# Angtian/VoGE

Measured on AMD Instinct MI355X. Metric: forward+backward frames/sec at 512^2, 50k Gaussians; ray-trace HBM GB/s vs peak, higher is better.
Workload: dtype f32; 1 GPU; cfg3_50k_512: 50000 random Gaussians (scalar sigmas), 512x512, K=40, max_point_per_bin=-1, fwd+bwd (grads to verts, sigmas, colors); launch=hip graph replay, 4 consecutive steps per graph launch, parallelism=1 gpu

## Files before the change

voge_amd/csrc/sweep_iso.h:

```cpp
#pragma once
#include <type_traits>

#include "voge_common.h"

namespace voge {

constexpr int kS2TP = 65;
constexpr int kS2TQ = 66;
constexpr int kS2Pad = 4;

struct Sweep2Stage {
  float x[64 + kS2Pad], y[64 + kS2Pad], z[64 + kS2Pad], a[64 + kS2Pad];
  union {
    float lb[64];
    int cnt[64];
  };
  int pos[64 + kS2Pad];
};
__host__ __device__ constexpr size_t sweep2_len_bytes(const int K) { return (sizeof(float) * (size_t)(K + 1) * kS2TP + 15) & ~(size_t)15; }
__host__ __device__ constexpr size_t sweep2_pos_bytes(const int K) { return (sizeof(uint16_t) * (size_t)(K + 1) * kS2TQ + 15) & ~(size_t)15; }
struct Sweep2Gen {
  float e[11][64 + kS2Pad];
};
constexpr int kS2DiagRows = 5;
__host__ __device__ constexpr size_t sweep2_lds_bytes(const int K, const int gen = 0) {
  return sweep2_len_bytes(K) + sweep2_pos_bytes(K) + sizeof(Sweep2Stage) +
         (gen == 1 ? sizeof(Sweep2Gen) : (gen == 2 ? sizeof(float) * kS2DiagRows * (64 + kS2Pad) : 0));
}

#ifndef VOGE_S2_EPI_B
#define VOGE_S2_EPI_B 5
#endif
#ifndef VOGE_S2_EPI_R
#define VOGE_S2_EPI_R 3
#endif
#ifndef VOGE_S2_EXIT_GROUP
#define VOGE_S2_EXIT_GROUP 16
#endif
constexpr int kExitGroup = VOGE_S2_EXIT_GROUP;

template <int GEN>
__global__ void __launch_bounds__(64)
sweep_iso_kernel(const float4 *__restrict__ cull, const float4 *__restrict__ ms, const float4 *__restrict__ evr, const float *__restrict__ rays,
                 const int *__restrict__ bin_count, const int32_t *__restrict__ bin_id, const float *__restrict__ bin_lb,
                 const int32_t *__restrict__ tl_id, const float *__restrict__ tl_lb, const int32_t *__restrict__ pool_id,
                 const float *__restrict__ pool_lb, const int *__restrict__ tl_off, const int2 *__restrict__ order,
                 const int tiles_per_img, const int nstx, const int nst, const int N, const int H, const int W, const int K,
                 const float thr_act, int32_t *__restrict__ out_idx, float *__restrict__ out_len, float *__restrict__ out_act,
                 float *__restrict__ out_dsd, int32_t *__restrict__ out_cnt,
                 const CamView cam ) {
  extern __shared__ __attribute__((aligned(16))) unsigned char smem_raw[];
  float *const Llen = reinterpret_cast<float *>(smem_raw);
  unsigned char *const Lpos_raw = smem_raw + sweep2_len_bytes(K);
  Sweep2Stage &S = *reinterpret_cast<Sweep2Stage *>(smem_raw + sweep2_len_bytes(K) + sweep2_pos_bytes(K));
  Sweep2Gen &G = *reinterpret_cast<Sweep2Gen *>(smem_raw + sweep2_len_bytes(K) + sweep2_pos_bytes(K) + sizeof(Sweep2Stage));
  auto grow = [&](const int r) -> float * { return &G.e[GEN == 2 ? (r < 2 ? r : r - 3) : r][0]; };
  auto ghas = [](const int r) { return GEN != 2 || r < 2 || (r >= 5 && r < 8); };

  const int lane = threadIdx.x;
  const int tiles_x = (W + 7) >> 3;
#ifdef VOGE_SWEEP_TIMES
  const unsigned long long ts0 = wall_clock64();
  unsigned long long ts_fill = 0, ts_cons = 0, ts1 = 0, ts2 = 0;
  unsigned st_eval = 0;
  unsigned long long ts_slow = 0; unsigned st_slow = 0, st_lanes = 0, st_moved = 0, st_far = 0;
  int dbg_moved = 0;
#endif
  const int2 slot = order[blockIdx.x];
  if (slot.x < 0) return;
  if (slot.y == 0) {
    if (out_act != nullptr) return;
    const int lin0 = slot.x & ~kPoolFlag;
    const int b = lin0 / tiles_per_img, bx = lin0 - b * tiles_per_img;
    const int ftx = bx % tiles_x, fty = bx / tiles_x;
    const int tw = min(8, W - ftx * 8), th = min(8, H - fty * 8);
    const int row_items = tw * K;
    if ((K & 3) == 0) {
      const int ipr = row_items >> 2;
      for (int it = lane; it < th * ipr; it += 64) {
        const int rr = it / ipr, j4 = it - rr * ipr;
        const size_t o = (((size_t)b * H + fty * 8 + rr) * W + (size_t)ftx * 8) * K + (size_t)j4 * 4;
        st16i<true>(out_idx + o, -1, -1, -1, -1);
        st16f<true>(out_len + o, VOGE_SENT_LEN, VOGE_SENT_LEN, VOGE_SENT_LEN, VOGE_SENT_LEN);
      }
    } else {
      for (int it = lane; it < th * row_items; it += 64) {
        const int rr = it / row_items, j = it - rr * row_items;
        const size_t o = (((size_t)b * H + fty * 8 + rr) * W + (size_t)ftx * 8) * K + j;
        out_idx[o] = -1; out_len[o] = VOGE_SENT_LEN;
      }
    }
    if (out_cnt != nullptr) {
      const int rr = lane >> 3, x = lane & 7;
      if (rr < th && x < tw) out_cnt[((size_t)b * H + fty * 8 + rr) * W + (size_t)ftx * 8 + x] = 0;
// ... 7 lines not shown
        float *o = cam.rays_out + (((size_t)b * H + fty * 8 + rr) * W + (size_t)ftx * 8 + x) * 3;
        o[0] = ex; o[1] = ey; o[2] = ez;
      }
    }
    return;
  }
  const bool pooled = (slot.x & kPoolFlag) != 0;
  const int lin = slot.x & ~kPoolFlag;
  const int b = lin / tiles_per_img, bx = lin - b * tiles_per_img;
  const int tx = bx % tiles_x, ty = bx / tiles_x;
  const int bin = (b * nst + ((ty * 8) / kST) * nstx + (tx * 8) / kST) * 4 + (((ty * 8) / kQuad) & 1) * 2 + (((tx * 8) / kQuad) & 1);
  const int tc = slot.y;
  const int bc = (tc >= 0) ? tc : ((bin_count != nullptr) ? bin_count[bin] : -1);
  const bool binned = bc >= 0;
  const int src_n = binned ? bc : N;
  const size_t list_at = pooled ? (size_t)tl_off[lin] : (size_t)lin * kTileCap;
  const int32_t *src_id = (tc >= 0) ? (pooled ? pool_id : tl_id) + list_at : (binned ? bin_id + (size_t)bin * kQCap : nullptr);
  const float *src_lb = (tc >= 0) ? (pooled ? pool_lb : tl_lb) + list_at : (binned ? bin_lb + (size_t)bin * kQCap : nullptr);
  const bool pref = tc >= 0;
  const float4 *cullb = cull + (size_t)b * N;
  const float4 *msb = ms + (size_t)b * N;
  const float4 rec_none = make_float4(0.f, 0.f, 0.f, INFINITY);
  const float4 cull_none = make_float4(0.f, 0.f, 0.f, -1.f);
  const bool h_is_id = (N <= 65536) || !binned;
  auto id_of = [&](const unsigned h) -> int { return h_is_id ? (int)h : src_id[h]; };
  const float not_full = __uint_as_float(__float_as_uint(VOGE_SENT_LEN) - 1u);
  if (lane < kS2Pad) { S.x[64 + lane] = 0.f; S.y[64 + lane] = 0.f; S.z[64 + lane] = 0.f; S.a[64 + lane] = INFINITY; }
  if (GEN && lane < kS2Pad) G.e[0][64 + lane] = __uint_as_float(0x7fc00000u);
  const float4 *evrb = GEN ? evr + (size_t)b * N * 3 : nullptr;
  bool tile_gen = false;

  Cone wcone;
  bool unit_rays = false;
  wcone.ok = false;
  const bool from_cam = cam.R != nullptr;
  CamK ck;
  if (from_cam) ck = cam_load(cam, b);
  auto ray_of = [&](const int x, const int y, float &rx, float &ry, float &rz) {
    if (from_cam) {
      cam_ray(ck, cam_irow(cam, y), x, rx, ry, rz);
    } else {
      const size_t rid = ((size_t)b * H + y) * W + x;
      rx = rays[3 * rid + 0]; ry = rays[3 * rid + 1]; rz = rays[3 * rid + 2];
    }
  };
  auto ray_setup = [&](const bool mine, const float mdx, const float mdy, const float mdz) {
    const int px = tx * 8 + (lane & 7), py = ty * 8 + (lane >> 3);
    float ox_ = mdx, oy_ = mdy, oz_ = mdz;
    if (!mine) ray_of(min(px, W - 1), min(py, H - 1), ox_, oy_, oz_);
    const RayDir u = ray_dir(ox_, oy_, oz_);
    unit_rays = __all(!u.ok || u.unit);
    wcone.ok = false;
    if (!pref) {
      const bool dirs_ok = __all(u.ok);
      const float wsx = wave_sum_dpp(u.ok ? u.ux : 0.f), wsy = wave_sum_dpp(u.ok ? u.uy : 0.f), wsz = wave_sum_dpp(u.ok ? u.uz : 0.f);
      const float n = sqrtf(fmaf(wsz, wsz, fmaf(wsy, wsy, wsx * wsx)));
      const float ax = wsx / n, ay = wsy / n, az = wsz / n;
      float smax = 0.f, cmin = 1.f;
      cone_partial(u, ax, ay, az, smax, cmin);
      wcone = cone_finish(ax, ay, az, n, wave_max(smax), wave_min(cmin), dirs_ok);
    }
  };

  auto run = [&](auto wide_tag, const int pass) {
    constexpr bool WIDE = decltype(wide_tag)::value;
    const int r = WIDE ? pass * 32 + (lane & 31) : lane;
    const int col = WIDE ? (lane & 31) : lane;
    const int px = tx * 8 + (r & 7), py = ty * 8 + (r >> 3);
    const bool valid = (px < W) && (py < H) && (!WIDE || lane < 32);
    const size_t ray_id = ((size_t)b * H + min(py, H - 1)) * W + min(px, W - 1);
    int id0 = (lane < src_n) ? (binned ? src_id[lane] : lane) : -1;
    float lb0 = (binned && lane < src_n) ? src_lb[lane] : -INFINITY;
    int id1 = (64 + lane < src_n) ? (binned ? src_id[64 + lane] : 64 + lane) : -1;
    float lb1 = (binned && 64 + lane < src_n) ? src_lb[64 + lane] : -INFINITY;
    float dx, dy, dz;
    ray_of(min(px, W - 1), min(py, H - 1), dx, dy, dz);
    if (from_cam && cam.rays_out != nullptr && valid) {
      float *o = cam.rays_out + 3 * ray_id;
      o[0] = dx; o[1] = dy; o[2] = dz;
    }
    const __amdgpu_buffer_rsrc_t rs_ms = out_rsrc(const_cast<float4 *>(msb), (unsigned)N * 16u),
                                 rs_cull = out_rsrc(const_cast<float4 *>(cullb), (unsigned)N * 16u);
    auto load_ms = [&](const int id) {
      const voge_v4f r = __builtin_amdgcn_raw_buffer_load_b128(rs_ms, id * 16, 0, 0);
      return make_float4(r[0], r[1], r[2], (id >= 0) ? r[3] : INFINITY);
    };
    auto load_cull = [&](const int id) {
      const voge_v4f r = __builtin_amdgcn_raw_buffer_load_b128(rs_cull, id * 16, 0, 0);
      return make_float4(r[0], r[1], r[2], (id >= 0) ? r[3] : -1.f);
    };
    const __amdgpu_buffer_rsrc_t rs_ev = out_rsrc(const_cast<float4 *>(GEN ? evrb : msb), GEN ? (unsigned)N * 48u : 0u);
    auto load_ev = [&](const int id, const int k) {
      const voge_v4f r = __builtin_amdgcn_raw_buffer_load_b128(rs_ev, id * 48 + 16 * k, 0, 0);
      return make_float4(r[0], r[1], r[2], r[3]);
    };
    float4 m0 = load_ms(id0);
    float4 c0 = pref ? cull_none : load_cull(id0);
    float4 ea0 = rec_none, ea1 = rec_none, ea2 = rec_none;
    if (GEN) { ea0 = load_ev(id0, 0); ea1 = load_ev(id0, 1); ea2 = load_ev(id0, 2); }
    if (pass == 0) ray_setup(!WIDE, dx, dy, dz);
    const float rdn2 = __builtin_amdgcn_rcpf((dx * dx + dy * dy) + dz * dz);
    float *const mylen = Llen + col;
// ... 333 lines not shown
        Pn = *reinterpret_cast<const int4 *>(&S.pos[s0 + 4]);
        if (GEN && chunk_diag) {
#pragma unroll
          for (int r = 0; r < 11; ++r)
            if (r < 2 || (r >= 5 && r < 8)) Evn[GEN ? r : 0] = *reinterpret_cast<const float4 *>(grow(r) + s0 + 4);
        } else if (GEN == 1 && gmask != 0ull) {
#pragma unroll
          for (int r = 0; r < 11; ++r) Evn[GEN ? r : 0] = *reinterpret_cast<const float4 *>(&G.e[r][s0 + 4]);
        }
#pragma unroll
        for (int q = 0; q < 4; ++q) commit(len[q], act[q], (unsigned)pv[q]);
      }
#ifdef VOGE_SWEEP_TIMES
      ts_cons += wall_clock64() - tsb;
      st_eval += min(n, nbuf);
#endif
    }
#ifdef VOGE_SWEEP_TIMES
    ts2 = wall_clock64();
#endif

    __syncthreads();
    S.cnt[lane] = valid ? cnt : 0;
    if (out_cnt != nullptr && valid) out_cnt[((size_t)b * H + py) * W + px] = cnt;
    __syncthreads();
    const int row0 = WIDE ? pass * 4 : 0;
    const int th = max(0, min(WIDE ? 4 : 8, H - ty * 8 - row0)), tw = min(8, W - tx * 8);
    const int row_items = tw * K;
    const uint16_t *const P16 = reinterpret_cast<const uint16_t *>(Lpos_raw);
    const uint32_t *const P32 = reinterpret_cast<const uint32_t *>(Lpos_raw);
    auto entry_pos = [&](const int s, const int owner) -> unsigned {
      return WIDE ? P32[s * (kS2TQ / 2) + owner] : (unsigned)P16[s * kS2TQ + owner];
    };
    const bool want_ad = out_act != nullptr;
    const int gofs = b * N;
    if ((K & 3) == 0) {
      constexpr int kEpiB = VOGE_S2_EPI_B, kEpiR = VOGE_S2_EPI_R;
      const int ipr = row_items >> 2, nitem = th * ipr;
      const float inv_ipr = 1.0f / (float)max(ipr, 1), invK = 1.0f / (float)K;
      const size_t tile_pix = ((size_t)b * H + ty * 8 + row0) * W + (size_t)tx * 8;
      int32_t *const t_idx = out_idx + tile_pix * K;
      float *const t_len = out_len + tile_pix * K;
      const unsigned h_last = (unsigned)max(src_n - 1, 0);
      const bool wt_ok = (size_t)W * (size_t)K < ((size_t)1 << 26);
      const unsigned rs_bytes = wt_ok ? (unsigned)th * (unsigned)W * (unsigned)K * 4u : 0u;
      const __amdgpu_buffer_rsrc_t rs_idx = out_rsrc(t_idx, rs_bytes), rs_len = out_rsrc(t_len, rs_bytes);
      for (int it0 = lane; it0 < nitem; it0 += 64 * kEpiB) {
        int32_t oi[kEpiB][4];
        float ol[kEpiB][4];
        unsigned rel[kEpiB];
        int nv[kEpiB];
#pragma unroll
        for (int u = 0; u < kEpiB; ++u) {
          const int it = it0 + u * 64;
          const bool in = it < nitem;
          const int itc = in ? it : 0;
          const int rr = __float2int_rz(((float)itc + 0.5f) * inv_ipr);
          const int j = (itc - rr * ipr) * 4;
          const int x = __float2int_rz(((float)j + 0.5f) * invK);
          const int sl = j - x * K;
          const int owner = rr * 8 + x;
          rel[u] = (unsigned)(rr * W + x) * (unsigned)K + (unsigned)sl;
          nv[u] = in ? max(0, min(4, S.cnt[owner] - sl)) : -1;
#pragma unroll
          for (int q = 0; q < 4; ++q) {
            const float l = Llen[(sl + q) * kS2TP + owner];
            const unsigned h = entry_pos(sl + q, owner);
// ... 147 lines not shown
#pragma unroll
          for (int u = 0; u < kOddU; ++u) {
            const float *ry = rays + (tile_pix + pr[u]) * 3;
            const float ex = ry[0], ey = ry[1], ez = ry[2];
            const size_t gi = (size_t)(in[u] ? oi[u] : gofs);
            const float4 cc = ms[gi];
            PairOut o;
            if (GEN && tile_gen && !(cc.w == cc.w)) {
              o = pair_eval_gen(cc.x, cc.y, cc.z, unpack_eval(evr[gi * 3], evr[gi * 3 + 1], evr[gi * 3 + 2]), ex, ey, ez, ex * ex, ey * ey,
                                ez * ez, ex * ey, ex * ez, ey * ez);
            } else {
              o = pair_eval_iso_at(cc.x, cc.y, cc.z, cc.w, ol[u], ex, ey, ez, (ex * ex + ey * ey) + ez * ez);
            }
            oa[u] = in[u] ? o.act : VOGE_SENT_ACT; od[u] = in[u] ? o.dsd : 0.0f;
          }
#pragma unroll
          for (int u = 0; u < kOddU; ++u)
            if (on[u]) { t_idx[rel[u]] = oi[u]; t_len[rel[u]] = ol[u]; t_act[rel[u]] = oa[u]; t_dsd[rel[u]] = od[u]; }
        }
      }
    }
  };

  if ((h_is_id ? N : src_n) <= 65536) {
    run(std::false_type{}, 0);
  } else {
    run(std::true_type{}, 0);
    run(std::true_type{}, 1);
  }
#ifdef VOGE_SWEEP_TIMES
  if (lane == 0 && b == 0 && bx < 8192) {
    unsigned long long *o = g_sweep_times + 8 * (size_t)bx;
    o[0] = ts0; o[1] = ts1; o[2] = ts_fill; o[3] = ts_cons; o[4] = ts2; o[5] = wall_clock64(); o[6] = ((unsigned long long)blockIdx.x << 32) | st_eval;
#ifdef VOGE_SWEEP_SLOW
    o[7] = (ts_slow << 32) | st_slow;
    o[2] = ((unsigned long long)st_far << 48) | ((unsigned long long)(st_moved & 0xffffu) << 32) | st_lanes;
#else
    o[7] = (unsigned long long)__builtin_amdgcn_s_getreg((4 << 0) | (0 << 6) | (31 << 11)) |
           ((unsigned long long)__builtin_amdgcn_s_getreg((20 << 0) | (0 << 6) | (31 << 11)) << 32);
#endif
  }
#endif
}

}
```

voge_amd/csrc/trace_bin.h:

```cpp
#pragma once
#include <type_traits>

#include "voge_common.h"

namespace voge {

constexpr int kST0 = 128;
constexpr int kCh = kST0 / kST;
constexpr int kBinThreads = 1024;
constexpr int kParts = 16;
constexpr int kSegCap = 512;
constexpr int kTileCap = 2048;
constexpr int kTilesPerBin = (kST / 8) * (kST / 8);
constexpr int kRankMaxBins = 4096;
static_assert(kCh * kCh == kBinThreads / 64, "one wave per super-tile of a region / per sweep tile of a super-tile");

__device__ __forceinline__ float depth_key(const float4 c, const Cone &k) {
  const float nm = __builtin_amdgcn_sqrtf(fmaf(c.z, c.z, fmaf(c.y, c.y, c.x * c.x)));
  const float R = c.w;
  if (!(R < 3e38f) || !(nm < 3e38f)) return -INFINITY;
  float kappa = -nm;
  if (k.ok && k.cs >= 0.5f && nm > 4.0f * R) {
    const float p = fmaf(c.z, k.az, fmaf(c.y, k.ay, c.x * k.ax));
    if (p > 0.0f) kappa = nm;
// ... 118 lines not shown
            const CamView cam ) {
  __shared__ BinALds L;
  const int tid = threadIdx.x, lane = tid & 63, wave = tid >> 6;
  const int region = blockIdx.x / kParts, part = blockIdx.x - region * kParts;
  const int b = blockIdx.y;
  if (blockIdx.x == 0 && blockIdx.y == 0 && tid == 0) *pool_top = 0ull;
  const int rx = region % nst0x, ry = region / nst0x;
  const int nst = nstx * nsty;
  if (tid < kCh * kCh) { L.base[tid] = 0; L.extn[tid] = 0; }
  if (tid == 0) L.arena_top = 0;
  int32_t *const arena = ext_id + ((size_t)(b * (int)(gridDim.x / kParts) + region) * kParts + part) * (size_t)ext_arena;
  int ext_have = 0;
  BIN_TS(0, 0);
  const bool interleaved = deal_interleaved(N);
  const int nchunks = interleaved ? kParts * ((N + kParts * kBinThreads - 1) / (kParts * kBinThreads))
                                  : (N + kBinThreads - 1) / kBinThreads;
  const bool writes_records = ISO_PREP && region == 0;
  float4 c[kRoundChunks];
  float av[kRoundChunks];
  int gq[kRoundChunks];
  CamK ck;
  if (cam.R != nullptr) ck = cam_load(cam, b);
  const BinAView V = binA_view<ISO_PREP>(b, cam_fwd, view, cam, &ck);
  if (cam.R != nullptr && cam.origin_out != nullptr && blockIdx.x == 0 && tid == 0) {
    float ox = V.ox, oy = V.oy, oz = V.oz;
    if (!ISO_PREP) cam_origin(ck, cam.T + 3 * b, ox, oy, oz);
    cam.origin_out[3 * b] = ox; cam.origin_out[3 * b + 1] = oy; cam.origin_out[3 * b + 2] = oz;
  }
  BinARaw raw[kRoundChunks];
  auto fetch_round = [&](const int j0) {
#pragma unroll
    for (int q = 0; q < kRoundChunks; ++q) {
      const int j = j0 + q * kParts;
      const int g = interleaved ? ((j / kParts) * kBinThreads + tid) * kParts + part : j * kBinThreads + tid;
      gq[q] = (j < nchunks && g < N) ? g : -1;
      raw[q] = binA_fetch<ISO_PREP>(gq[q], b, N, cull, mus, isg, view);
    }
  };
  auto derive_round = [&]() {
#pragma unroll
    for (int q = 0; q < kRoundChunks; ++q) c[q] = binA_derive<ISO_PREP>(raw[q], gq[q] >= 0, V, thr_act, view, av[q]);
  };
  auto load_round = [&](const int j0) { fetch_round(j0); derive_round(); };
  fetch_round(part);
  if (wave == 0) {
    const int cc = lane & (kCh * kCh - 1);
    const int cx = rx * kCh + (cc & (kCh - 1)), cy = ry * kCh + cc / kCh;
    ConeRec r = {0.f, 0.f, 1.f, 1.f, 0.f, -1.f, 0.f, 0.f};
    const bool region_rect = cam.R != nullptr && cam.h <= cam.stripe_h;
    if (cam.R != nullptr) {
      const bool reg = region_rect && lane == kCh * kCh;
      const int j0 = reg ? rx * kCh * kST : cx * kST, i0 = reg ? ry * kCh * kST : cy * kST, ext = reg ? kCh * kST : kST;
      if ((cx < nstx && cy < nsty) || reg) r = cam_rect_cone(ck, cam, j0, j0 + ext - 1, i0, i0 + ext - 1);
    } else if (cx < nstx && cy < nsty) {
      r = cones[cone_super_at(b, nst, cy * nstx + cx)];
    }
    if (lane < kCh * kCh) L.child[lane] = r;
    if (region_rect) {
      if (lane == kCh * kCh) L.region = r;
      if (lane == 0) L.use_rows = 0;
    } else {
    const bool present = lane < kCh * kCh && r.ok >= 0.f;
    const float sx = wave_sum_dpp(present ? r.ax : 0.f), sy = wave_sum_dpp(present ? r.ay : 0.f), sz = wave_sum_dpp(present ? r.az : 0.f);
    const float npres = wave_sum_dpp(present ? 1.f : 0.f);
    bool ok = __all(!present || r.ok > 0.f);
    const float n = sqrtf(fmaf(sz, sz, fmaf(sy, sy, sx * sx)));
    const float ax = sx / n, ay = sy / n, az = sz / n;
    auto child_extrema = [&](const float ax_, const float ay_, const float az_, float &smax_, float &cmin_, bool &ok_) {
      smax_ = 0.f; cmin_ = 1.f;
      if (present) {
        const float ca = fmaf(r.az, az_, fmaf(r.ay, ay_, r.ax * ax_));
        const float qx = fmaf(-ca, ax_, r.ax), qy = fmaf(-ca, ay_, r.ay), qz = fmaf(-ca, az_, r.az);
        const float sa = sqrtf(fmaf(qz, qz, fmaf(qy, qy, qx * qx))) * (1.0f + 1e-6f) + 1e-7f;
        const float cl = fminf(ca, 1.0f) - 1e-7f;
        if (!(cl > 0.0f)) ok_ = false;
        cmin_ = fmaf(cl, r.cs, -sa * r.sn);
        smax_ = fmaf(fminf(ca + 1e-7f, 1.0f), r.sn, sa);
      }
    };
    float smax, cmin;
    child_extrema(ax, ay, az, smax, cmin, ok);
    ok = __all(ok);
    smax = wave_max(smax); cmin = wave_min(cmin);
    const Cone cn = cone_finish(ax, ay, az, n / fmaxf(npres, 1.f), smax, cmin, ok);
    if (lane == 0) L.region = ConeRec{cn.ax, cn.ay, cn.az, cn.cs, cn.sn, cn.ok ? 1.f : 0.f, 0.f, 0.f};
    const float widest_child = wave_max(present ? (r.ok > 0.f ? r.sn : 2.0f) : 0.f);
    if (lane == 0) L.use_rows = 0;
    if (__builtin_expect((!cn.ok || cn.sn > 8.0f * widest_child) && N < (1 << 27), 0)) {
      auto quad_sum = [](float v) { v += VOGE_DPP(v, 0xB1); v += VOGE_DPP(v, 0x4E); return v; };
      auto quad_max = [](float v) { v = fmaxf(v, VOGE_DPP(v, 0xB1)); v = fmaxf(v, VOGE_DPP(v, 0x4E)); return v; };
      auto quad_min = [](float v) { v = fminf(v, VOGE_DPP(v, 0xB1)); v = fminf(v, VOGE_DPP(v, 0x4E)); return v; };
      static_assert(kCh == 4, "a row of super-tiles is a DPP quad");
      const float qsx = quad_sum(present ? r.ax : 0.f), qsy = quad_sum(present ? r.ay : 0.f), qsz = quad_sum(present ? r.az : 0.f);
      const float qn = quad_sum(present ? 1.f : 0.f);
      const float nn = sqrtf(fmaf(qsz, qsz, fmaf(qsy, qsy, qsx * qsx)));
      const float rax = qsx / nn, ray = qsy / nn, raz = qsz / nn;
      float rs, rc;
      bool rok = !present || r.ok > 0.f;
      child_extrema(rax, ray, raz, rs, rc, rok);
      rs = quad_max(rs); rc = quad_min(rc);
      const float okf = quad_min(rok ? 1.f : 0.f);
      const Cone rcn = cone_finish(rax, ray, raz, nn / fmaxf(qn, 1.f), rs, rc, okf != 0.f);
      if (lane < kCh * kCh && (lane & 3) == 0) L.rowc[lane >> 2] = ConeRec{rcn.ax, rcn.ay, rcn.az, rcn.cs, rcn.sn, qn > 0.f ? (rcn.ok ? 1.f : 0.f) : -1.f, 0.f, 0.f};
      const float widest_row = wave_max((lane < kCh * kCh && qn > 0.f) ? (rcn.ok ? rcn.sn : 2.0f) : 0.f);
      if (lane == 0) L.use_rows = (!cn.ok || cn.sn > 1.6f * widest_row) ? 1 : 0;
    }
    }
  }
  BIN_TS(0, 6);
  derive_round();
  BIN_TS(0, 7);
  __syncthreads();
  const Cone rcone = load_cone(L.region);
  const bool use_rows = L.use_rows != 0;
  BIN_TS(0, 1);

  auto rounds = [&](auto rows_tag) {
    constexpr bool ROWS = decltype(rows_tag)::value;
    for (int j0 = part; j0 < nchunks; j0 += kParts * kRoundChunks) {
      if (j0 != part) load_round(j0);
      bool k0[kRoundChunks];
      unsigned rowm[kRoundChunks];
  #pragma unroll
      for (int q = 0; q < kRoundChunks; ++q) {
        if (writes_records && gq[q] >= 0) {
// ... 246 lines not shown
      }
      bin_test_batch<ELL>(S, gid, c, sink);
    }
  }
}
__device__ __forceinline__ void bin_batch_slots(int *count , const int lane, const bool (&kp)[kGU], int (&slot)[kGU]) {
  unsigned long long m[kGU];
  int cw = 0;
#pragma unroll
  for (int j = 0; j < kGU; ++j) { m[j] = __ballot(kp[j]); cw += __popcll(m[j]); }
  int start = 0;
  if (cw > 0) {
    if (lane == 0) start = atomicAdd(count, cw);
    start = __builtin_amdgcn_readfirstlane(start);
  }
#pragma unroll
  for (int j = 0; j < kGU; ++j) {
    slot[j] = start + __popcll(m[j] & ((1ull << lane) - 1ull));
    start += __popcll(m[j]);
  }
}
struct BinKeys {
  float lo, scale, span, slack;
  bool flagged;
};
__device__ __forceinline__ int bin_bucket_of(const BinKeys &Kk, const float v) {
  return (v > -INFINITY) ? 1 + min(kBuckets - 2, max(0, (int)((v - Kk.lo) * Kk.scale))) : 0;
}
__device__ __forceinline__ float bin_own_bound(const BinStream &S, const size_t g) {
  const float4 cj = S.cullb[g], e0 = S.ellb[2 * g], e1 = S.ellb[2 * g + 1];
  float bnd = -INFINITY;
  if (S.qcone.ok) {
    const float pa = fmaf(cj.z, S.qcone.az, fmaf(cj.y, S.qcone.ay, cj.x * S.qcone.ax));
    const float nm1 = fabsf(cj.x) + fabsf(cj.y) + fabsf(cj.z);
    const float t = pa - ell_support(e0, e1, S.qcone.ax, S.qcone.ay, S.qcone.az) - 4e-6f * nm1;
    bnd = (t >= 0.0f) ? t : t / S.qcone.cs;
    bnd = bnd - 1e-5f * fabsf(bnd) - 1e-30f;
  }
  return bnd;
}
__device__ __forceinline__ void bin_bmin_suffix(uint32_t *bmin, int *wsum, const int tid) {
  const int lane = tid & 63, wave = tid >> 6;
  uint32_t m4[2];
#pragma unroll
  for (int q = 0; q < 2; ++q) m4[q] = bmin[2 * tid + q];
  m4[0] = min(m4[0], m4[1]);
  uint32_t x = m4[0];
#pragma unroll
  for (int o = 1; o < 64; o <<= 1) {
    const uint32_t y = __shfl_down(x, o, 64);
    if (lane + o < 64) x = min(x, y);
  }
  if (lane == 0) wsum[4 + wave] = (int)x;
  __syncthreads();
  uint32_t later = 0xffffffffu;
  {
    const uint32_t nxt = __shfl_down(x, 1, 64);
    later = (lane < 63) ? nxt : 0xffffffffu;
    for (int w = wave + 1; w < 4; ++w) later = min(later, (uint32_t)wsum[4 + w]);
  }
#pragma unroll
  for (int q = 0; q < 2; ++q) bmin[2 * tid + q] = min(m4[q], later);
}
__device__ __forceinline__ float bin_len_bound(const BinKeys &Kk, const uint32_t *bmin, const float v) {
  float edge = -INFINITY;
  int qb = 0;
  if (v > -INFINITY) {
    const int q = min(kBuckets - 2, max(0, (int)((v - Kk.lo) * Kk.scale)));
    edge = fminf(v, Kk.lo + (float)q * (Kk.span / (float)(kBuckets - 2)) - 4e-6f * Kk.span);
    qb = 1 + q;
  }
  const float lb_sphere = (edge > -INFINITY) ? edge - Kk.slack - 1e-5f * fabsf(edge) - 1e-30f : -INFINITY;
  return Kk.flagged ? fminf(lb_sphere, ord2f(bmin[qb])) : lb_sphere;
}

struct BinLong {
  BinStream S;
  BinKeys Kk;
  Cone tcone;
  bool tile_ok;
  int tile, quad, total;
  unsigned long long *pool_top;
  int *tl_off, *tl_count, *q_count;
  const int *seg_ext;
  int bin;
  int pool_cap;
  int32_t *pool_id;
  float *pool_lb;
  int2 *my_order;
};
template <bool ELL>
__device__ __forceinline__ void binB_long_path(const BinLong A, BinLds &L) {
// ... 252 lines not shown
        if (!el[j] && cj[j].w < 3e38f) rmax = fmaxf(rmax, cj[j].w);
        const float kv = el[j] ? gkey[j] : depth_key(cj[j], qcone);
        if (kv > -INFINITY) { klo = fminf(klo, kv); khi = fmaxf(khi, kv); }
        if (slot[j] < kQCap) L.keys[slot[j]] = ((uint64_t)f2ord(kv) << 32) | (uint32_t)g[j] | (el[j] ? 0x80000000u : 0u);
        any_el = any_el || el[j];
      }
    }
  });
  BIN_TS(1, 1);
  if (__any(any_el) && lane == 0) L.nflag = 1;
  float hi = wave_max(khi), lo = wave_min(klo), rm = wave_max(rmax);
  if (lane == 0) { L.red[wave * 8 + 0] = hi; L.red[wave * 8 + 1] = lo; L.red[wave * 8 + 2] = rm; }
  if (S.n_ext > 0) __syncthreads();
  for (int i = tid; i < kBuckets; i += kQT) { L.hist[i] = 0; L.bmin[i] = f2ord(INFINITY); }
  __syncthreads();
  const int total = L.count;
  hi = fmaxf(fmaxf(L.red[0], L.red[8]), fmaxf(L.red[16], L.red[24]));
  lo = fminf(fminf(L.red[1], L.red[9]), fminf(L.red[17], L.red[25]));
  rm = fmaxf(fmaxf(L.red[2], L.red[10]), fmaxf(L.red[18], L.red[26]));
  const float span = fmaxf(hi - lo, 1e-20f);
  const float scale = (float)(kBuckets - 2) / span;
  const bool flagged = ELL && L.nflag != 0;
  BinKeys Kk;
  Kk.lo = lo; Kk.scale = scale; Kk.span = span; Kk.slack = 1.13f * rm * (1.0f + 1e-5f); Kk.flagged = flagged;
  auto bucket_of = [&](const uint64_t k) { return bin_bucket_of(Kk, ord2f((uint32_t)(k >> 32))); };
  if (__builtin_expect(total > kQCap, 0)) {
    BinLong A;
    A.S = S; A.Kk = Kk; A.tcone = tcone; A.tile_ok = tile_ok; A.tile = tile; A.quad = quad; A.total = total;
    A.pool_top = pool_top; A.tl_off = tl_off; A.tl_count = tl_count; A.q_count = q_count; A.pool_cap = pool_cap;
    A.pool_id = pool_id; A.pool_lb = pool_lb; A.my_order = my_order; A.seg_ext = seg_ext; A.bin = bin;
    binB_long_path<ELL>(A, L);
  } else {
  for (int i = tid; i < total; i += kQT) {
    const uint64_t kk = L.keys[i];
    const int q = bucket_of(kk);
    atomicAdd(&L.hist[q], 1);
    if (ELL && ((uint32_t)kk & 0x80000000u)) atomicMin(&L.bmin[q], f2ord(bin_own_bound(S, (size_t)((uint32_t)kk & 0x7fffffffu))));
  }
  __syncthreads();
  {
    static_assert(kBuckets == 2 * kQT, "two buckets per thread");
    const int2 v = *reinterpret_cast<const int2 *>(&L.hist[2 * tid]);
    const int s4 = v.x + v.y;
    int x = s4;
#pragma unroll
    for (int o = 1; o < 64; o <<= 1) {
      const int y = __shfl_up(x, o, 64);
// ... 155 lines not shown
```

voge_amd/csrc/trace_fwd.hip:

```cpp
#include "voge_common.h"

namespace voge {

__device__ inline double lambda_min_sym3(double a00, double a11, double a22, double a01,
                                         double a02, double a12) {
  const double p1 = a01 * a01 + a02 * a02 + a12 * a12;
  if (p1 == 0.0) return fmin(a00, fmin(a11, a22));
  const double q = (a00 + a11 + a22) / 3.0;
  const double b00 = a00 - q, b11 = a11 - q, b22 = a22 - q;
  const double p2 = b00 * b00 + b11 * b11 + b22 * b22 + 2.0 * p1;
  const double p = sqrt(p2 / 6.0);
  const double ip = 1.0 / p;
  const double c00 = b00 * ip, c11 = b11 * ip, c22 = b22 * ip;
  const double c01 = a01 * ip, c02 = a02 * ip, c12 = a12 * ip;
  double r = 0.5 * (c00 * (c11 * c22 - c12 * c12) - c01 * (c01 * c22 - c12 * c02) +
                    c02 * (c01 * c12 - c11 * c02));
  r = fmin(1.0, fmax(-1.0, r));
  const double phi = acos(r) / 3.0;
  return q + 2.0 * p * cos(phi + 2.0943951023931953);
}

__device__ __forceinline__ void prep_one(const int g, const float *__restrict__ mus, const float *__restrict__ isg,
                                         const float *__restrict__ cam_fwd, const int N, const float thr_act,
                                         const int iso_in, float4 *__restrict__ cull, float4 *__restrict__ evr,
// ... 307 lines not shown
    ws->tl_lb = reinterpret_cast<float *>(tl);
    ws->seg_rec = reinterpret_cast<float4 *>(sr); ws->order = reinterpret_cast<int2 *>(cq);
    ws->nstx = nstx; ws->nsty = nsty;
    ws->nst0x = (W + kST0 - 1) / kST0; ws->nst0y = (H + kST0 - 1) / kST0;
    ws->nbin = (int)nbin;
  }
  return off;
}

}
#ifdef VOGE_AB
#include "sweep_r3.h"
#else
namespace voge { constexpr bool ab_round3_selected() { return false; } }
#endif
namespace voge {

template <bool ISO>
static int launch_trace(const TraceWs &ws, const ConeRec *cones, const float *rays, int B, int N, int H, int W, int K,
                        float thr_act, int32_t *idx, float *len, float *act, float *dsd, int32_t *cnt, hipStream_t st,
                        const CamView &cam, const bool diag = false) {
  constexpr int T = 64;
  const int gen = ISO ? 0 : (diag ? 2 : 1);
  const auto sweep = ISO ? sweep_iso_kernel<0> : (diag ? sweep_iso_kernel<2> : sweep_iso_kernel<1>);
  const bool v2 = !ab_round3_selected();
  const size_t lds2 = sweep2_lds_bytes(K, gen);
  {
    static DynLdsCache cache2[2];
    if (v2) {
      const int rc = ensure_dynamic_lds(reinterpret_cast<const void *>(sweep), lds2, cache2[diag ? 1 : 0]);
      if (rc) return rc;
    }
  }
  hipLaunchKernelGGL(binB_kernel<!ISO>, dim3(ws.nstx * ws.nsty * 4, B), dim3(kQT), 0, st, ws.cull, ws.ell, ws.seg_count, ws.seg_id, ws.seg_rec,
                     cones, N, H, W, ws.nstx, ws.nsty, ws.nbin, ws.q_count, ws.q_id, ws.q_lb, ws.tl_count, ws.tl_id, ws.tl_lb,
                     ws.order, ws.pool_top, ws.pool_cap, ws.pool_id, ws.pool_lb, ws.tl_off, ws.seg_ext, ws.ext_id, K,
                     (v2 && act == nullptr) ? nullptr : idx , len, act, dsd, cnt,
                     nullptr, nullptr, cam);
  {
    int rc = launch_status();
    if (rc) return rc;
  }
  dim3 grid(ws.nbin * kTilesPerBin);
#ifdef VOGE_AB
  if (!v2) return launch_sweep_r3<ISO>(ws, rays, grid, N, H, W, K, thr_act, idx, len, act, dsd, cnt, st, cam);
#endif
  hipLaunchKernelGGL(sweep, grid, dim3(T), lds2, st, ws.cull, ws.ms, ws.evr, rays, ws.q_count, ws.q_id, ws.q_lb, ws.tl_id,
                     ws.tl_lb, ws.pool_id, ws.pool_lb, ws.tl_off, ws.order, ((W + 7) / 8) * ((H + 7) / 8), ws.nstx, ws.nstx * ws.nsty, N, H, W, K,
                     thr_act, idx, len, act, dsd, cnt, cam);
  return launch_status();
}

}
// ... 367 lines not shown
```

voge_amd/csrc/voge_common.h:

```cpp
#pragma once
#include <hip/hip_runtime.h>
#include <stdint.h>

#include <atomic>
#include <type_traits>

#include "voge_hip.h"

#define VOGE_WAVE 64

#define VOGE_SENT_LEN 1e10f
#define VOGE_SENT_ACT 1e10f

namespace voge {

struct EvalRec {
  float s00, s11, s22, s01, s02, s12;
  float bx, by, bz;
  float kx, ky, kz;
};
static_assert(sizeof(EvalRec) == 48, "EvalRec must be 3 x float4");

__device__ __forceinline__ float fast_div(const float a, const float b) { return a * __builtin_amdgcn_rcpf(b); }

// ... 331 lines not shown
  float ax, ay, az, cs, sn;
  bool ok;
};

__device__ __forceinline__ bool cone_keep(const float4 c, const Cone &k) {
  if (c.w < 0.0f) return false;
  const float p = fmaf(c.z, k.az, fmaf(c.y, k.ay, c.x * k.ax));
  const float rx = fmaf(-p, k.ax, c.x), ry = fmaf(-p, k.ay, c.y), rz = fmaf(-p, k.az, c.z);
  const float q = __builtin_amdgcn_sqrtf(fmaf(rz, rz, fmaf(ry, ry, rx * rx)));
  const float gap = fmaf(q, k.cs, -fabsf(p) * k.sn);
  return !k.ok || !(gap > c.w);
}

constexpr int kST = 32;

struct RayDir {
  float ux, uy, uz;
  bool ok;
  bool unit;
};
__device__ __forceinline__ RayDir ray_dir(const float dx, const float dy, const float dz) {
  RayDir r;
  const float dn2 = fmaf(dz, dz, fmaf(dy, dy, dx * dx));
  const float inv = 1.0f / sqrtf(dn2);
  r.ok = (dn2 > 0.0f) && (inv < 3e38f) && (inv == inv);
  r.unit = fabsf(dn2 - 1.0f) < 1e-4f;
  r.ux = dx * inv; r.uy = dy * inv; r.uz = dz * inv;
  return r;
}
__device__ __forceinline__ void cone_partial(const RayDir &u, const float ax, const float ay, const float az,
                                             float &smax, float &cmin) {
  const float cl = fmaf(u.uz, az, fmaf(u.uy, ay, u.ux * ax));
  const float rx = fmaf(-cl, ax, u.ux), ry = fmaf(-cl, ay, u.uy), rz = fmaf(-cl, az, u.uz);
  const float sl = sqrtf(fmaf(rz, rz, fmaf(ry, ry, rx * rx)));
  smax = fmaxf(smax, u.ok ? sl : 2.0f);
  cmin = fminf(cmin, u.ok ? cl : -1.0f);
}
__device__ __forceinline__ Cone cone_finish(const float ax, const float ay, const float az, const float n,
                                            const float smax, const float cmin, const bool all_ok) {
  Cone c;
  c.ax = ax; c.ay = ay; c.az = az;
  c.sn = smax * (1.0f + 1e-5f) + 1e-7f;
  c.cs = cmin - 1e-6f;
  c.ok = all_ok && (n > 1e-3f) && (cmin > 0.05f) && (c.sn == c.sn);
  return c;
}

struct ConeRec {
  float ax, ay, az, cs, sn, ok, pad0, pad1;
};
__device__ __forceinline__ Cone load_cone(const ConeRec &r) {
  Cone c;
  c.ax = r.ax; c.ay = r.ay; c.az = r.az; c.cs = r.cs; c.sn = r.sn; c.ok = r.ok > 0.f;
  return c;
}

struct Mat3 {
  float m[9];
};
__device__ __forceinline__ Mat3 inv3(const float *R) {
  Mat3 o;
  const float a = R[0], b = R[1], c = R[2], d = R[3], e = R[4], f = R[5], g = R[6], h = R[7], i = R[8];
  const float A = e * i - f * h, B = -(d * i - f * g), C = d * h - e * g;
  const float det = a * A + b * B + c * C;
  const float id = 1.0f / det;
  o.m[0] = A * id;               o.m[1] = -(b * i - c * h) * id;  o.m[2] = (b * f - c * e) * id;
// ... 178 lines not shown
      const float4 v = L.sum[i];
      const float c = L.cnt[i];
      vx += in ? v.x : 0.f; vy += in ? v.y : 0.f; vz += in ? v.z : 0.f;
      ok = (in && c > 0.f) ? fminf(ok, v.w) : ok;
      n_in += in ? c : 0.f;
      const float e_s = level == 0 ? L.ext[i][0] : L.ext[i][2];
      const float e_c = level == 0 ? L.ext[i][1] : L.ext[i][3];
      s2 = (in && c > 0.f && level != 1) ? fmaxf(s2, e_s) : s2;
      cm = (in && c > 0.f && level != 1) ? fminf(cm, e_c) : cm;
    }
    const float n2 = fmaf(vz, vz, fmaf(vy, vy, vx * vx)), rn = __builtin_amdgcn_rsqf(n2);
    const float Ax = vx * rn, Ay = vy * rn, Az = vz * rn;
    float smax = sqrtf(s2) * (1.0f + 4e-7f) + 4e-7f, cmin = cm - 4e-7f;
    bool all_ok = ok != 0.f;
    if (level == 1) {
      smax = 0.f; cmin = 1.f;
#pragma unroll
      for (int k = 0; k < 4; ++k) {
        const int i = q0 + (k >> 1) * 4 + (k & 1);
        if (!(L.cnt[i] > 0.f)) continue;
        const float4 v = L.sum[i];
        const float trn = __builtin_amdgcn_rsqf(fmaf(v.z, v.z, fmaf(v.y, v.y, v.x * v.x)));
        const float tx = v.x * trn, ty = v.y * trn, tz = v.z * trn;
        const float t_sn = (sqrtf(L.ext[i][0]) * (1.0f + 4e-7f) + 4e-7f) * (1.0f + 1e-5f) + 1e-7f;
        const float t_cs = (L.ext[i][1] - 4e-7f) - 1e-6f;
        const float ca = fmaf(tz, Az, fmaf(ty, Ay, tx * Ax));
        const float qx = fmaf(-ca, Ax, tx), qy = fmaf(-ca, Ay, ty), qz = fmaf(-ca, Az, tz);
        const float sa = sqrtf(fmaf(qz, qz, fmaf(qy, qy, qx * qx))) * (1.0f + 1e-6f) + 1e-7f;
        const float cl = fminf(ca, 1.0f) - 1e-7f;
        if (!(cl > 0.0f) || !(t_cs > 0.0f)) all_ok = false;
        cmin = fminf(cmin, fmaf(cl, t_cs, -sa * t_sn));
        smax = fmaxf(smax, fmaf(fminf(ca + 1e-7f, 1.0f), t_sn, sa));
      }
    }
    const Cone c = cone_finish(Ax, Ay, Az, (n2 * rn) / fmaxf(n_in, 1.f), smax, cmin, all_ok);
    const ConeRec rec = {c.ax, c.ay, c.az, c.cs, c.sn, n_in > 0.f ? (c.ok ? 1.f : 0.f) : -1.f, 0.f, 0.f};
    if (level == 0) c_tile[t] = rec; else if (level == 1) c_quad[t - 16] = rec; else *c_super = rec;
  }
}

__device__ __forceinline__ ConeRec cam_rect_cone(const CamK &k, const CamView &c, int j0, int j1, int i0, int i1) {
  if (j0 >= c.W || i0 >= c.h || j1 < j0 || i1 < i0) return ConeRec{0.f, 0.f, 1.f, 1.f, 0.f, -1.f, 0.f, 0.f};
  j1 = min(j1, c.W - 1); i1 = min(i1, c.h - 1);
  const int r0 = cam_irow(c, i0), r1 = cam_irow(c, i1);
  float ux[4], uy[4], uz[4];
  cam_ray(k, r0, j0, ux[0], uy[0], uz[0]); cam_ray(k, r0, j1, ux[1], uy[1], uz[1]);
  cam_ray(k, r1, j0, ux[2], uy[2], uz[2]); cam_ray(k, r1, j1, ux[3], uy[3], uz[3]);
  const float sx = (ux[0] + ux[1]) + (ux[2] + ux[3]), sy = (uy[0] + uy[1]) + (uy[2] + uy[3]), sz = (uz[0] + uz[1]) + (uz[2] + uz[3]);
// ... 320 lines not shown
```

Baseline: 4653 frames/s.

## Specialize iso sweep kernel for frame layout and small N; use fast rsq/sqrt intrinsics

Adds FRAME and HID template specializations of the iso sweep kernel. They compile out the activation/dsd epilogue, drop the id indirection and the wide two-pass path when N is at most 65536, and use byte-offset buffer stores for the ray and count outputs. Separately, divisions and sqrtf in the cone construction and ray normalization become hardware rsq/sqrt/rcp intrinsics, with cone error margins widened to cover the lower precision. A bucket step is precomputed in BinKeys. The wider margins may loosen culling slightly, and the approximate intrinsics change rounding.

```diff
diff --git a/voge_amd/csrc/sweep_iso.h b/voge_amd/csrc/sweep_iso.h
--- a/voge_amd/csrc/sweep_iso.h
+++ b/voge_amd/csrc/sweep_iso.h
@@ -1,6 +1,7 @@
 #pragma once
 #include <type_traits>
 
+#include "composite_core.h"
 #include "voge_common.h"
 
 namespace voge {
@@ -39,7 +40,7 @@
 #endif
 constexpr int kExitGroup = VOGE_S2_EXIT_GROUP;
 
-template <int GEN>
+template <int GEN, bool FRAME = false, bool HID = false>
 __global__ void __launch_bounds__(64)
 sweep_iso_kernel(const float4 *__restrict__ cull, const float4 *__restrict__ ms, const float4 *__restrict__ evr, const float *__restrict__ rays,
                  const int *__restrict__ bin_count, const int32_t *__restrict__ bin_id, const float *__restrict__ bin_lb,
@@ -69,7 +70,7 @@
   const int2 slot = order[blockIdx.x];
   if (slot.x < 0) return;
   if (slot.y == 0) {
-    if (out_act != nullptr) return;
+    if (!FRAME && out_act != nullptr) return;
     const int lin0 = slot.x & ~kPoolFlag;
     const int b = lin0 / tiles_per_img, bx = lin0 - b * tiles_per_img;
     const int ftx = bx % tiles_x, fty = bx / tiles_x;
@@ -123,7 +124,7 @@
   const float4 *msb = ms + (size_t)b * N;
   const float4 rec_none = make_float4(0.f, 0.f, 0.f, INFINITY);
   const float4 cull_none = make_float4(0.f, 0.f, 0.f, -1.f);
-  const bool h_is_id = (N <= 65536) || !binned;
+  const bool h_is_id = HID || (N <= 65536) || !binned;
   auto id_of = [&](const unsigned h) -> int { return h_is_id ? (int)h : src_id[h]; };
   const float not_full = __uint_as_float(__float_as_uint(VOGE_SENT_LEN) - 1u);
   if (lane < kS2Pad) { S.x[64 + lane] = 0.f; S.y[64 + lane] = 0.f; S.z[64 + lane] = 0.f; S.a[64 + lane] = INFINITY; }
@@ -155,11 +156,11 @@
     if (!pref) {
       const bool dirs_ok = __all(u.ok);
       const float wsx = wave_sum_dpp(u.ok ? u.ux : 0.f), wsy = wave_sum_dpp(u.ok ? u.uy : 0.f), wsz = wave_sum_dpp(u.ok ? u.uz : 0.f);
-      const float n = sqrtf(fmaf(wsz, wsz, fmaf(wsy, wsy, wsx * wsx)));
-      const float ax = wsx / n, ay = wsy / n, az = wsz / n;
+      const float n2 = fmaf(wsz, wsz, fmaf(wsy, wsy, wsx * wsx)), rn = __builtin_amdgcn_rsqf(n2);
+      const float ax = wsx * rn, ay = wsy * rn, az = wsz * rn;
       float smax = 0.f, cmin = 1.f;
       cone_partial(u, ax, ay, az, smax, cmin);
-      wcone = cone_finish(ax, ay, az, n, wave_max(smax), wave_min(cmin), dirs_ok);
+      wcone = cone_finish(ax, ay, az, n2 * rn, wave_max(smax), wave_min(cmin), dirs_ok);
     }
   };
 
@@ -176,9 +177,16 @@
     float lb1 = (binned && 64 + lane < src_n) ? src_lb[64 + lane] : -INFINITY;
     float dx, dy, dz;
     ray_of(min(px, W - 1), min(py, H - 1), dx, dy, dz);
+    const size_t tile_pix0 = ((size_t)b * H + ty * 8) * W + (size_t)tx * 8;
+    const unsigned pix_rel = (unsigned)(r >> 3) * (unsigned)W + (unsigned)(r & 7);
     if (from_cam && cam.rays_out != nullptr && valid) {
-      float *o = cam.rays_out + 3 * ray_id;
-      o[0] = dx; o[1] = dy; o[2] = dz;
+      if constexpr (FRAME) {
+        float *const o = cam.rays_out + 3 * tile_pix0;
+        at_bytes_w<float>(o, pix_rel * 12u) = dx; at_bytes_w<float>(o, pix_rel * 12u + 4u) = dy; at_bytes_w<float>(o, pix_rel * 12u + 8u) = dz;
+      } else {
+        float *o = cam.rays_out + 3 * ray_id;
+        o[0] = dx; o[1] = dy; o[2] = dz;
+      }
     }
     const __amdgpu_buffer_rsrc_t rs_ms = out_rsrc(const_cast<float4 *>(msb), (unsigned)N * 16u),
                                  rs_cull = out_rsrc(const_cast<float4 *>(cullb), (unsigned)N * 16u);
@@ -558,7 +566,10 @@
 
     __syncthreads();
     S.cnt[lane] = valid ? cnt : 0;
-    if (out_cnt != nullptr && valid) out_cnt[((size_t)b * H + py) * W + px] = cnt;
+    if (out_cnt != nullptr && valid) {
+      if constexpr (FRAME) at_bytes_w<int32_t>(out_cnt + tile_pix0, pix_rel * 4u) = cnt;
+      else out_cnt[((size_t)b * H + py) * W + px] = cnt;
+    }
     __syncthreads();
     const int row0 = WIDE ? pass * 4 : 0;
     const int th = max(0, min(WIDE ? 4 : 8, H - ty * 8 - row0)), tw = min(8, W - tx * 8);
@@ -568,7 +579,7 @@
     auto entry_pos = [&](const int s, const int owner) -> unsigned {
       return WIDE ? P32[s * (kS2TQ / 2) + owner] : (unsigned)P16[s * kS2TQ + owner];
     };
-    const bool want_ad = out_act != nullptr;
+    const bool want_ad = !FRAME && out_act != nullptr;
     const int gofs = b * N;
     if ((K & 3) == 0) {
       constexpr int kEpiB = VOGE_S2_EPI_B, kEpiR = VOGE_S2_EPI_R;
@@ -578,7 +589,7 @@
       int32_t *const t_idx = out_idx + tile_pix * K;
       float *const t_len = out_len + tile_pix * K;
       const unsigned h_last = (unsigned)max(src_n - 1, 0);
-      const bool wt_ok = (size_t)W * (size_t)K < ((size_t)1 << 26);
+      const bool wt_ok = FRAME || (size_t)W * (size_t)K < ((size_t)1 << 26);
       const unsigned rs_bytes = wt_ok ? (unsigned)th * (unsigned)W * (unsigned)K * 4u : 0u;
       const __amdgpu_buffer_rsrc_t rs_idx = out_rsrc(t_idx, rs_bytes), rs_len = out_rsrc(t_len, rs_bytes);
       for (int it0 = lane; it0 < nitem; it0 += 64 * kEpiB) {
@@ -772,11 +783,15 @@
     }
   };
 
-  if ((h_is_id ? N : src_n) <= 65536) {
+  if constexpr (HID) {
     run(std::false_type{}, 0);
   } else {
-    run(std::true_type{}, 0);
-    run(std::true_type{}, 1);
+    if ((h_is_id ? N : src_n) <= 65536) {
+      run(std::false_type{}, 0);
+    } else {
+      run(std::true_type{}, 0);
+      run(std::true_type{}, 1);
+    }
   }
 #ifdef VOGE_SWEEP_TIMES
   if (lane == 0 && b == 0 && bx < 8192) {
diff --git a/voge_amd/csrc/trace_bin.h b/voge_amd/csrc/trace_bin.h
--- a/voge_amd/csrc/trace_bin.h
+++ b/voge_amd/csrc/trace_bin.h
@@ -164,7 +164,7 @@
   CamK ck;
   if (cam.R != nullptr) ck = cam_load(cam, b);
   const BinAView V = binA_view<ISO_PREP>(b, cam_fwd, view, cam, &ck);
-  if (cam.R != nullptr && cam.origin_out != nullptr && blockIdx.x == 0 && tid == 0) {
+  if ((ISO_PREP || N <= 0) && cam.R != nullptr && cam.origin_out != nullptr && blockIdx.x == 0 && tid == 0) {
     float ox = V.ox, oy = V.oy, oz = V.oz;
     if (!ISO_PREP) cam_origin(ck, cam.T + 3 * b, ox, oy, oz);
     cam.origin_out[3 * b] = ox; cam.origin_out[3 * b + 1] = oy; cam.origin_out[3 * b + 2] = oz;
@@ -206,25 +206,25 @@
     const float sx = wave_sum_dpp(present ? r.ax : 0.f), sy = wave_sum_dpp(present ? r.ay : 0.f), sz = wave_sum_dpp(present ? r.az : 0.f);
     const float npres = wave_sum_dpp(present ? 1.f : 0.f);
     bool ok = __all(!present || r.ok > 0.f);
-    const float n = sqrtf(fmaf(sz, sz, fmaf(sy, sy, sx * sx)));
-    const float ax = sx / n, ay = sy / n, az = sz / n;
+    const float n2 = fmaf(sz, sz, fmaf(sy, sy, sx * sx)), rn = __builtin_amdgcn_rsqf(n2);
+    const float ax = sx * rn, ay = sy * rn, az = sz * rn;
     auto child_extrema = [&](const float ax_, const float ay_, const float az_, float &smax_, float &cmin_, bool &ok_) {
       smax_ = 0.f; cmin_ = 1.f;
       if (present) {
         const float ca = fmaf(r.az, az_, fmaf(r.ay, ay_, r.ax * ax_));
         const float qx = fmaf(-ca, ax_, r.ax), qy = fmaf(-ca, ay_, r.ay), qz = fmaf(-ca, az_, r.az);
-        const float sa = sqrtf(fmaf(qz, qz, fmaf(qy, qy, qx * qx))) * (1.0f + 1e-6f) + 1e-7f;
-        const float cl = fminf(ca, 1.0f) - 1e-7f;
+        const float sa = __builtin_amdgcn_sqrtf(fmaf(qz, qz, fmaf(qy, qy, qx * qx))) * (1.0f + 1e-6f) + 4e-7f;
+        const float cl = fminf(ca, 1.0f) - 4e-7f;
         if (!(cl > 0.0f)) ok_ = false;
         cmin_ = fmaf(cl, r.cs, -sa * r.sn);
-        smax_ = fmaf(fminf(ca + 1e-7f, 1.0f), r.sn, sa);
+        smax_ = fmaf(fminf(ca + 4e-7f, 1.0f), r.sn, sa);
       }
     };
     float smax, cmin;
     child_extrema(ax, ay, az, smax, cmin, ok);
     ok = __all(ok);
     smax = wave_max(smax); cmin = wave_min(cmin);
-    const Cone cn = cone_finish(ax, ay, az, n / fmaxf(npres, 1.f), smax, cmin, ok);
+    const Cone cn = cone_finish(ax, ay, az, n2 * rn * __builtin_amdgcn_rcpf(fmaxf(npres, 1.f)), smax, cmin, ok);
     if (lane == 0) L.region = ConeRec{cn.ax, cn.ay, cn.az, cn.cs, cn.sn, cn.ok ? 1.f : 0.f, 0.f, 0.f};
     const float widest_child = wave_max(present ? (r.ok > 0.f ? r.sn : 2.0f) : 0.f);
     if (lane == 0) L.use_rows = 0;
@@ -235,14 +235,14 @@
       static_assert(kCh == 4, "a row of super-tiles is a DPP quad");
       const float qsx = quad_sum(present ? r.ax : 0.f), qsy = quad_sum(present ? r.ay : 0.f), qsz = quad_sum(present ? r.az : 0.f);
       const float qn = quad_sum(present ? 1.f : 0.f);
-      const float nn = sqrtf(fmaf(qsz, qsz, fmaf(qsy, qsy, qsx * qsx)));
-      const float rax = qsx / nn, ray = qsy / nn, raz = qsz / nn;
+      const float nn2 = fmaf(qsz, qsz, fmaf(qsy, qsy, qsx * qsx)), rnn = __builtin_amdgcn_rsqf(nn2);
+      const float rax = qsx * rnn, ray = qsy * rnn, raz = qsz * rnn;
       float rs, rc;
       bool rok = !present || r.ok > 0.f;
       child_extrema(rax, ray, raz, rs, rc, rok);
       rs = quad_max(rs); rc = quad_min(rc);
       const float okf = quad_min(rok ? 1.f : 0.f);
-      const Cone rcn = cone_finish(rax, ray, raz, nn / fmaxf(qn, 1.f), rs, rc, okf != 0.f);
+      const Cone rcn = cone_finish(rax, ray, raz, nn2 * rnn * __builtin_amdgcn_rcpf(fmaxf(qn, 1.f)), rs, rc, okf != 0.f);
       if (lane < kCh * kCh && (lane & 3) == 0) L.rowc[lane >> 2] = ConeRec{rcn.ax, rcn.ay, rcn.az, rcn.cs, rcn.sn, qn > 0.f ? (rcn.ok ? 1.f : 0.f) : -1.f, 0.f, 0.f};
       const float widest_row = wave_max((lane < kCh * kCh && qn > 0.f) ? (rcn.ok ? rcn.sn : 2.0f) : 0.f);
       if (lane == 0) L.use_rows = (!cn.ok || cn.sn > 1.6f * widest_row) ? 1 : 0;
@@ -535,6 +535,7 @@
 }
 struct BinKeys {
   float lo, scale, span, slack;
+  float step;
   bool flagged;
 };
 __device__ __forceinline__ int bin_bucket_of(const BinKeys &Kk, const float v) {
@@ -580,7 +581,7 @@
   int qb = 0;
   if (v > -INFINITY) {
     const int q = min(kBuckets - 2, max(0, (int)((v - Kk.lo) * Kk.scale)));
-    edge = fminf(v, Kk.lo + (float)q * (Kk.span / (float)(kBuckets - 2)) - 4e-6f * Kk.span);
+    edge = fminf(v, Kk.lo + (float)q * Kk.step - 4e-6f * Kk.span);
     qb = 1 + q;
   }
   const float lb_sphere = (edge > -INFINITY) ? edge - Kk.slack - 1e-5f * fabsf(edge) - 1e-30f : -INFINITY;
@@ -879,7 +880,7 @@
   const float scale = (float)(kBuckets - 2) / span;
   const bool flagged = ELL && L.nflag != 0;
   BinKeys Kk;
-  Kk.lo = lo; Kk.scale = scale; Kk.span = span; Kk.slack = 1.13f * rm * (1.0f + 1e-5f); Kk.flagged = flagged;
+  Kk.lo = lo; Kk.scale = scale; Kk.span = span; Kk.step = span / (float)(kBuckets - 2); Kk.slack = 1.13f * rm * (1.0f + 1e-5f); Kk.flagged = flagged;
   auto bucket_of = [&](const uint64_t k) { return bin_bucket_of(Kk, ord2f((uint32_t)(k >> 32))); };
   if (__builtin_expect(total > kQCap, 0)) {
     BinLong A;
diff --git a/voge_amd/csrc/trace_fwd.hip b/voge_amd/csrc/trace_fwd.hip
--- a/voge_amd/csrc/trace_fwd.hip
+++ b/voge_amd/csrc/trace_fwd.hip
@@ -353,13 +353,16 @@
                         const CamView &cam, const bool diag = false) {
   constexpr int T = 64;
   const int gen = ISO ? 0 : (diag ? 2 : 1);
-  const auto sweep = ISO ? sweep_iso_kernel<0> : (diag ? sweep_iso_kernel<2> : sweep_iso_kernel<1>);
+  const bool frame = ISO && act == nullptr && (size_t)W * (size_t)(K > 3 ? K : 3) < ((size_t)1 << 26);
+  const bool hid = N <= 65536;
+  const auto sweep = ISO ? (frame ? (hid ? sweep_iso_kernel<0, true, true> : sweep_iso_kernel<0, true, false>) : sweep_iso_kernel<0>)
+                         : (diag ? sweep_iso_kernel<2> : sweep_iso_kernel<1>);
   const bool v2 = !ab_round3_selected();
   const size_t lds2 = sweep2_lds_bytes(K, gen);
   {
-    static DynLdsCache cache2[2];
+    static DynLdsCache cache2[3];
     if (v2) {
-      const int rc = ensure_dynamic_lds(reinterpret_cast<const void *>(sweep), lds2, cache2[diag ? 1 : 0]);
+      const int rc = ensure_dynamic_lds(reinterpret_cast<const void *>(sweep), lds2, cache2[ISO ? (frame ? (hid ? 2 : 1) : 0) : (diag ? 1 : 0)]);
       if (rc) return rc;
     }
   }
diff --git a/voge_amd/csrc/voge_common.h b/voge_amd/csrc/voge_common.h
--- a/voge_amd/csrc/voge_common.h
+++ b/voge_amd/csrc/voge_common.h
@@ -377,7 +377,7 @@
 __device__ __forceinline__ RayDir ray_dir(const float dx, const float dy, const float dz) {
   RayDir r;
   const float dn2 = fmaf(dz, dz, fmaf(dy, dy, dx * dx));
-  const float inv = 1.0f / sqrtf(dn2);
+  const float inv = __builtin_amdgcn_rsqf(dn2);
   r.ok = (dn2 > 0.0f) && (inv < 3e38f) && (inv == inv);
   r.unit = fabsf(dn2 - 1.0f) < 1e-4f;
   r.ux = dx * inv; r.uy = dy * inv; r.uz = dz * inv;
@@ -387,16 +387,18 @@
                                              float &smax, float &cmin) {
   const float cl = fmaf(u.uz, az, fmaf(u.uy, ay, u.ux * ax));
   const float rx = fmaf(-cl, ax, u.ux), ry = fmaf(-cl, ay, u.uy), rz = fmaf(-cl, az, u.uz);
-  const float sl = sqrtf(fmaf(rz, rz, fmaf(ry, ry, rx * rx)));
+  const float sl = __builtin_amdgcn_sqrtf(fmaf(rz, rz, fmaf(ry, ry, rx * rx)));
   smax = fmaxf(smax, u.ok ? sl : 2.0f);
   cmin = fminf(cmin, u.ok ? cl : -1.0f);
 }
+__device__ __forceinline__ float cone_sn_bound(const float smax) { return smax * (1.0f + 1e-5f) + 3.5e-7f; }
+__device__ __forceinline__ float cone_cs_bound(const float cmin) { return cmin - 1.25e-6f; }
 __device__ __forceinline__ Cone cone_finish(const float ax, const float ay, const float az, const float n,
                                             const float smax, const float cmin, const bool all_ok) {
   Cone c;
   c.ax = ax; c.ay = ay; c.az = az;
-  c.sn = smax * (1.0f + 1e-5f) + 1e-7f;
-  c.cs = cmin - 1e-6f;
+  c.sn = cone_sn_bound(smax);
+  c.cs = cone_cs_bound(cmin);
   c.ok = all_ok && (n > 1e-3f) && (cmin > 0.05f) && (c.sn == c.sn);
   return c;
 }
@@ -621,8 +623,8 @@
         const float4 v = L.sum[i];
         const float trn = __builtin_amdgcn_rsqf(fmaf(v.z, v.z, fmaf(v.y, v.y, v.x * v.x)));
         const float tx = v.x * trn, ty = v.y * trn, tz = v.z * trn;
-        const float t_sn = (sqrtf(L.ext[i][0]) * (1.0f + 4e-7f) + 4e-7f) * (1.0f + 1e-5f) + 1e-7f;
-        const float t_cs = (L.ext[i][1] - 4e-7f) - 1e-6f;
+        const float t_sn = cone_sn_bound(sqrtf(L.ext[i][0]) * (1.0f + 4e-7f) + 4e-7f);
+        const float t_cs = cone_cs_bound(L.ext[i][1] - 4e-7f);
         const float ca = fmaf(tz, Az, fmaf(ty, Ay, tx * Ax));
         const float qx = fmaf(-ca, Ax, tx), qy = fmaf(-ca, Ay, ty), qz = fmaf(-ca, Az, tz);
         const float sa = sqrtf(fmaf(qz, qz, fmaf(qy, qy, qx * qx))) * (1.0f + 1e-6f) + 1e-7f;
```

Measured after the change: 4693 frames/s, median of 6. Within noise of the previous version (+0.9%).
